# CrispyChillies/Image-Retrieval---Thesis-2026

Measured on AMD Instinct MI355X. Metric: queries/sec (embed+top-10) over 1M x 1024 gallery, higher is better.
Workload: dtype f32 embed (two fp16 MFMA terms); bf16 MFMA candidates + f64 re-rank

## Files before the change

image-retrieval---thesis-2026_amd/csrc/k_conv1x1_h2.hip:

```cpp
#include <atomic>

#include "mirx_device.h"
#include "mirx_kernels.h"

namespace mirx {

namespace {

#ifdef MIRX_C1H2_STAMPS
__device__ unsigned long long g_c1_stamps[8192 * 8];
#define C1_STAMP(ACC)                                                 \
    {                                                                 \
        const unsigned long long now_ = __builtin_amdgcn_s_memtime(); \
        ACC += now_ - st_t;                                           \
        st_t = now_;                                                  \
    }
#else
#define C1_STAMP(ACC)
#endif

constexpr int CM = 128;
constexpr int CP = 128;
constexpr int KC = 16;
constexpr int PLANE_A = CM * KC * 2;
constexpr int PLANE_B = CP * KC * 2;
#ifndef MIRX_C1H2_MIN_WG
#define MIRX_C1H2_MIN_WG 256
#endif
#ifndef MIRX_C1H2_NPT
#define MIRX_C1H2_NPT 2
#endif

__device__ __forceinline__ void pair_exchange(const u32x4 &p, const u32x4 &q, u32x4 &a, u32x4 &b) {
    unsigned a0, a1, a2, a3, b0, b1, b2, b3;
    asm volatile("s_nop 1\n"
                 "s_mov_b64 vcc, %[me]\n"
                 "v_cndmask_b32_dpp %[a0], %[q0], %[p0], vcc quad_perm:[1,0,3,2] row_mask:0xf bank_mask:0xf\n"
                 "v_cndmask_b32_dpp %[a1], %[q1], %[p1], vcc quad_perm:[1,0,3,2] row_mask:0xf bank_mask:0xf\n"
                 "v_cndmask_b32_dpp %[a2], %[q2], %[p2], vcc quad_perm:[1,0,3,2] row_mask:0xf bank_mask:0xf\n"
                 "v_cndmask_b32_dpp %[a3], %[q3], %[p3], vcc quad_perm:[1,0,3,2] row_mask:0xf bank_mask:0xf\n"
                 "s_mov_b64 vcc, %[mo]\n"
                 "v_cndmask_b32_dpp %[b0], %[p0], %[q0], vcc quad_perm:[1,0,3,2] row_mask:0xf bank_mask:0xf\n"
                 "v_cndmask_b32_dpp %[b1], %[p1], %[q1], vcc quad_perm:[1,0,3,2] row_mask:0xf bank_mask:0xf\n"
                 "v_cndmask_b32_dpp %[b2], %[p2], %[q2], vcc quad_perm:[1,0,3,2] row_mask:0xf bank_mask:0xf\n"
                 "v_cndmask_b32_dpp %[b3], %[p3], %[q3], vcc quad_perm:[1,0,3,2] row_mask:0xf bank_mask:0xf\n"
                 : [a0] "=&v"(a0), [a1] "=&v"(a1), [a2] "=&v"(a2), [a3] "=&v"(a3), [b0] "=&v"(b0), [b1] "=&v"(b1),
                   [b2] "=&v"(b2), [b3] "=&v"(b3)
                 : [p0] "v"(p[0]), [p1] "v"(p[1]), [p2] "v"(p[2]), [p3] "v"(p[3]), [q0] "v"(q[0]), [q1] "v"(q[1]),
                   [q2] "v"(q[2]), [q3] "v"(q[3]), [me] "s"(0x5555555555555555ull), [mo] "s"(0xaaaaaaaaaaaaaaaaull)
                 : "vcc");
    a = u32x4{a0, a1, a2, a3};
    b = u32x4{b0, b1, b2, b3};
}

#define C1H2_PARAMS                                                                                                      \
    const float *__restrict__ x, int64_t xbs, int cin, const float *__restrict__ scale, const float *__restrict__ shift, \
        const uint16_t *__restrict__ w2, const float *__restrict__ oscale, const float *__restrict__ bias, int64_t n,     \
        int hw, int cout, float *__restrict__ y, int64_t ybs, const float *__restrict__ in_amax, float in_ks, float in_kb, \
        unsigned *__restrict__ out_amax, float y_ks, float y_kb, float *__restrict__ y_inv_out, int64_t xps, int64_t yps
#define C1H2_ARGS x, xbs, cin, scale, shift, w2, oscale, bias, n, hw, cout, y, ybs, in_amax, in_ks, in_kb, out_amax, y_ks, y_kb, \
                  y_inv_out, xps, yps

template <bool PROLOGUE, bool RELU_OUT, bool YTERMS, int NPT, bool TABLED>
__device__ __forceinline__ void conv1x1_tiled(C1H2_PARAMS) {
    extern __shared__ __attribute__((aligned(16))) char sm[];
    constexpr int KIMG = 8;
    __shared__ float sBias[CM], sOsc[KIMG][CM];
    constexpr bool YFOLD = YTERMS && TABLED;
    __shared__ float sBiasY[YFOLD ? KIMG : 1][CM];
    const int wave = __builtin_amdgcn_readfirstlane(threadIdx.x >> 6), lane = threadIdx.x & 63;
    const int tid = threadIdx.x;
    const int wm = wave >> 1, wn = wave & 1;
    const int64_t total = n * (int64_t)hw;
    constexpr int STAGE_N = 2 * PLANE_A + NPT * 2 * PLANE_B;
    const int64_t p0 = (int64_t)blockIdx.x * (CP * NPT);
    const int co0 = blockIdx.y * CM;
    const int nk = cin / KC;

    auto image_bound = [&](int64_t img) { return fmaf(in_ks, in_amax ? in_amax[img] : 0.f, in_kb); };

    const int b_px = tid & 127;
    const int b_kg = wave >> 1;
    const int64_t in_hw = xps;
    const float *xsrc[NPT];
    float x_scale[NPT];
    unsigned st_img[NPT];
#pragma unroll
    for (int u = 0; u < NPT; ++u) {
        const unsigned pp = (unsigned)(p0 + u * CP + b_px);
        const bool live = pp < (unsigned)total;
        const unsigned pimg = (live ? pp : (unsigned)total - 1u) / (unsigned)hw;
        const int64_t b_off = live ? (int64_t)pimg * xbs + (pp - pimg * (unsigned)hw) : 0;
        st_img[u] = pimg;
        xsrc[u] = x + b_off + (int64_t)(8 * b_kg) * in_hw;
    }
#if defined(MIRX_C1H2_EXP_SKIP) && (MIRX_C1H2_EXP_SKIP & 32)
    const int b_row = b_px;
#else
    const int b_row = YTERMS ? ((b_px & ~31) | ((b_px & 15) << 1) | ((b_px >> 4) & 1)) : b_px;
#endif
    const int b_lds = 2 * PLANE_A + b_row * 32 + ((b_kg ^ ((b_row >> 3) & 1)) << 4);
    const int ep_px = YTERMS ? 16 * (lane & 1) + ((lane & 31) >> 1) : (lane & 31);
    const __amdgpu_buffer_rsrc_t wrsrc = __builtin_amdgcn_make_buffer_rsrc(
        (void *)(w2 + ((int64_t)blockIdx.y * nk) * (2 * CM * KC)), 0, nk * (2 * CM * KC * 2), 0x00020000);
    const int w_voff = (lane >> 1) * 32 + (((lane & 1) ^ ((lane >> 4) & 1)) << 4);
    [[maybe_unused]] auto dma_w1 = [&](int kt, int buf, int i) {
        const int piece = wave + 4 * i;
        __builtin_amdgcn_raw_ptr_buffer_load_lds(wrsrc, LDS_PTR(sm + buf * STAGE_N + piece * 1024), 16, w_voff,
                                                 kt * (2 * CM * KC * 2) + piece * 1024, 0, 0);
    };
    [[maybe_unused]] auto dma_w = [&](int kt, int buf) {
        dma_w1(kt, buf, 0);
        dma_w1(kt, buf, 1);
    };

    constexpr int NR = 8;
    float ra[NPT][NR], rb[NPT][NR], sca[8], sha[8], scb[8], shb[8];
    auto load = [&](int kt, float (&r)[NPT][NR], float (&rsc)[8], float (&rsh)[8]) {
#pragma unroll
        for (int u = 0; u < NPT; ++u)
#pragma unroll
            for (int j = 0; j < 8; ++j) {
                r[u][j] = xsrc[u][((int64_t)kt * KC + j) * in_hw];
            }
        if (PROLOGUE) {
#pragma unroll
            for (int j = 0; j < 8; ++j) {
                rsc[j] = scale[kt * KC + 8 * b_kg + j];
                rsh[j] = shift[kt * KC + 8 * b_kg + j];
            }
        }
    };
#ifdef MIRX_C1H2_STAMPS
    unsigned long long st_t = __builtin_amdgcn_s_memtime(), st_wait = 0, st_bar = 0, st_issue = 0, st_mfma = 0, st_store = 0, st_valu = 0;
    const unsigned long long st_begin = st_t, rt_begin = __builtin_amdgcn_s_memrealtime();
#endif
    auto store = [&](int buf, const float (&r)[NPT][NR], const float (&rsc)[8], const float (&rsh)[8]) {
        char *sb = sm + buf * STAGE_N;
#pragma unroll
        for (int u = 0; u < NPT; ++u) {
            u32x4 ph, pl;
#pragma unroll
            for (int j = 0; j < 4; ++j) {
                f32x2 v;
                v[0] = r[u][2 * j];
                v[1] = r[u][2 * j + 1];
                if (PROLOGUE) {
                    v[0] = fmaxf(fmaf(v[0], rsc[2 * j], rsh[2 * j]), 0.f);
                    v[1] = fmaxf(fmaf(v[1], rsc[2 * j + 1], rsh[2 * j + 1]), 0.f);
                }
                unsigned th, tl;
#if defined(MIRX_C1H2_EXP_SPLIT) && MIRX_C1H2_EXP_SPLIT == 0
                th = __float_as_uint(r[u][2 * j]);
                tl = __float_as_uint(r[u][2 * j + 1]);
#elif defined(MIRX_C1H2_EXP_SPLIT) && MIRX_C1H2_EXP_SPLIT == 1
                th = __float_as_uint(v[0] * x_scale[u]);
                tl = __float_as_uint(v[1] * x_scale[u]);
#else
                split2h_pair(v[0] * x_scale[u], v[1] * x_scale[u], th, tl);
#endif
                ph[j] = th;
                pl[j] = tl;
            }
#ifdef MIRX_C1H2_STAMPS
            if (u == NPT - 1) {
                __builtin_amdgcn_sched_barrier(0);
                asm volatile("s_waitcnt lgkmcnt(0)" ::: "memory");
                C1_STAMP(st_valu)
            }
#endif
            *reinterpret_cast<u32x4 *>(sb + b_lds + u * 2 * PLANE_B) = ph;
            *reinterpret_cast<u32x4 *>(sb + b_lds + u * 2 * PLANE_B + PLANE_B) = pl;
        }
    };

    const int kg = lane >> 5;
    constexpr int NN = 2 * NPT;
    int fa[2], fb[2];
#pragma unroll
    for (int t = 0; t < 2; ++t) {
        const int ra_ = wm * 64 + t * 32 + (lane & 31);
        fa[t] = ra_ * 32 + ((kg ^ ((ra_ >> 3) & 1)) << 4);
        const int rb_ = wn * 64 + t * 32 + (lane & 31);
        fb[t] = 2 * PLANE_A + rb_ * 32 + ((kg ^ ((rb_ >> 3) & 1)) << 4);
    }

    const unsigned img_first = (unsigned)(p0 < total ? p0 : total - 1) / (unsigned)hw;
    const unsigned p_last = (unsigned)(p0 + CP * NPT - 1 < total ? p0 + CP * NPT - 1 : total - 1);
    constexpr bool tabled = TABLED;

    f32x16 acc[2][NN];
#pragma unroll
    for (int mi = 0; mi < 2; ++mi)
#pragma unroll
        for (int ni = 0; ni < NN; ++ni)
#pragma unroll
            for (int r = 0; r < 16; ++r) acc[mi][ni][r] = 0.f;

    auto stage = [&](int kt, int cur, float (&rnext)[NPT][NR], float (&scn)[8], float (&shn)[8], const float (&rstore)[NPT][NR],
                     const float (&scs)[8], const float (&shs)[8]) {
        C1_STAMP(st_store)
        asm volatile("s_waitcnt vmcnt(0)" ::: "memory");
        C1_STAMP(st_wait)
        __syncthreads();
        C1_STAMP(st_bar)
#if defined(MIRX_C1H2_EXP_SKIP) && (MIRX_C1H2_EXP_SKIP & 1)
        if (kt < 0)
#endif
        dma_w(kt + 1 < nk ? kt + 1 : kt, cur ^ 1);
        __builtin_amdgcn_sched_barrier(0);
        load(kt + 2 < nk ? kt + 2 : nk - 1, rnext, scn, shn);
        __builtin_amdgcn_sched_barrier(0);
        C1_STAMP(st_issue)
        const char *sb = sm + cur * STAGE_N;
        f16x8 a[2][2], b[NN][2];
#pragma unroll
        for (int t = 0; t < 2; ++t)
#pragma unroll
            for (int p = 0; p < 2; ++p) a[t][p] = *reinterpret_cast<const f16x8 *>(sb + fa[t] + p * PLANE_A);
#pragma unroll
        for (int ni = 0; ni < NN; ++ni)
#pragma unroll
            for (int p = 0; p < 2; ++p)
                b[ni][p] = *reinterpret_cast<const f16x8 *>(sb + fb[ni & 1] + (ni >> 1) * 2 * PLANE_B + p * PLANE_B);
#pragma unroll
        for (int mi = 0; mi < 2; ++mi) {
#pragma unroll
            for (int ni = 0; ni < NN; ++ni) {
                f32x16 c = acc[mi][ni];
#ifndef MIRX_C1H2_EXP_ONE_MFMA
                c = __builtin_amdgcn_mfma_f32_32x32x16_f16(a[mi][1], b[ni][0], c, 0, 0, 0);
                c = __builtin_amdgcn_mfma_f32_32x32x16_f16(a[mi][0], b[ni][1], c, 0, 0, 0);
#endif
                c = __builtin_amdgcn_mfma_f32_32x32x16_f16(a[mi][0], b[ni][0], c, 0, 0, 0);
                acc[mi][ni] = c;
            }
        }
        C1_STAMP(st_mfma)
        store(cur ^ 1, rstore, scs, shs);
    };
    dma_w(0, 0);
    load(0, ra, sca, sha);
    load(nk > 1 ? 1 : 0, rb, scb, shb);
    if (tid < CM) {
        const float bias_v = bias ? bias[co0 + tid] : 0.f;
        sBias[tid] = bias_v;
        const float osc = oscale[co0 + tid];
        sOsc[0][tid] = osc;
        if (tabled) {
            const unsigned nimg = p_last / (unsigned)hw - img_first + 1;
            for (unsigned k = 0; k < nimg; ++k) {
                float xs_, xi_;
                const float xb_ = image_bound(img_first + k);
                range_scales(xb_, xs_, xi_);
                float ys_ = 1.f, yi_;
                if (YFOLD) range_scales(fmaf(y_ks, xb_, y_kb), ys_, yi_);
                sOsc[k][tid] = osc * xi_ * ys_;
                if (YFOLD) sBiasY[k][tid] = bias_v * ys_;
            }
        }
    }
#pragma unroll
    for (int u = 0; u < NPT; ++u) {
        float inv_;
        range_scales(image_bound(st_img[u]), x_scale[u], inv_);
    }
    float ep_xinv[NN], ep_ys[NN];
    int ep_k[NN];
#pragma unroll
    for (int ni = 0; ni < NN; ++ni) {
        unsigned pp = (unsigned)(p0 + (ni >> 1) * CP + wn * 64 + 32 * (ni & 1) + ep_px);
        if (pp >= (unsigned)total) pp = (unsigned)total - 1u;
        const unsigned pimg = pp / (unsigned)hw;
        const float xb = image_bound(pimg);
        float xs_, yi_;
        range_scales(xb, xs_, ep_xinv[ni]);
        ep_k[ni] = tabled ? (int)(pimg - img_first) : 0;
        if (tabled) ep_xinv[ni] = 1.f;
        ep_ys[ni] = 1.f;
        if (YTERMS) range_scales(fmaf(y_ks, xb, y_kb), ep_ys[ni], yi_);
    }

    store(0, ra, sca, sha);
    int kt = 0;
    for (; kt + 1 < nk; kt += 2) {
        stage(kt, 0, ra, sca, sha, rb, scb, shb);
        stage(kt + 1, 1, rb, scb, shb, ra, sca, sha);
    }
    if (kt < nk) stage(kt, 0, ra, sca, sha, rb, scb, shb);
#ifdef MIRX_C1H2_STAMPS
    if (threadIdx.x == 0) {
        const unsigned long long now_ = __builtin_amdgcn_s_memtime();
        unsigned long long *o = g_c1_stamps + ((blockIdx.x + blockIdx.y * gridDim.x) & 8191) * 8;
        o[0] = now_ - st_begin;
        o[1] = __builtin_amdgcn_s_memrealtime() - rt_begin;
        o[2] = nk;
        o[3] = st_wait;
        o[4] = st_bar;
        o[5] = st_issue;
        o[6] = st_mfma;
        o[7] = (st_store << 32) | (st_valu & 0xffffffffull);
    }
#endif

#if defined(MIRX_C1H2_EXP_SKIP) && (MIRX_C1H2_EXP_SKIP & 2)
    if (in_ks > -1e30f) return;
#endif
    if (YTERMS) {
        uint16_t *yt = reinterpret_cast<uint16_t *>(y);
        auto nb = [](unsigned v) { return (unsigned)__builtin_amdgcn_update_dpp(0, (int)v, 0xB1, 0xf, 0xf, true); };
        const bool even = !(lane & 1);
#pragma unroll
        for (int ni = 0; ni < NN; ++ni) {
            const unsigned pp = (unsigned)(p0 + (ni >> 1) * CP + wn * 64 + 32 * (ni & 1) + ep_px);
            const bool live = pp < (unsigned)total;
            const unsigned ubimg = (live ? pp : 0u) / (unsigned)hw;
            const int64_t bimg = ubimg;
            const unsigned off = pp - ubimg * (unsigned)hw;
            if (live && off == 0 && wm == 0 && lane < 32) {
                float ys_, y_inv;
                range_scales(fmaf(y_ks, image_bound(bimg), y_kb), ys_, y_inv);
                y_inv_out[bimg] = y_inv;
            }
            const unsigned q_own = live ? ubimg * 16u * (unsigned)hw + off : 0xffffffffu;
            const unsigned q_nb = nb(q_own);
            const unsigned qa = even ? q_own : q_nb, qb = even ? q_nb : q_own;
            [[maybe_unused]] const float x_inv = ep_xinv[ni], y_scale = ep_ys[ni];
#pragma unroll
            for (int mi = 0; mi < 2; ++mi) {
                const int g = 4 * wm + 2 * mi + (lane >> 5);
                u32x4 h0, h1, l0, l1;
#pragma unroll
                for (int j = 0; j < 8; ++j) {
                    f32x2 v;
#pragma unroll
                    for (int e = 0; e < 2; ++e) {
                        const int r = 2 * j + e;
                        const int ch = wm * 64 + mi * 32 + (r & 3) + 8 * (r >> 2) + 4 * (lane >> 5);
#if defined(MIRX_C1H2_EXP_SKIP) && (MIRX_C1H2_EXP_SKIP & 8)
                        v[e] = acc[mi][ni][r];
                        (void)ch;
#else
                        float t = fmaf(acc[mi][ni][r], TABLED ? sOsc[ep_k[ni]][ch] : sOsc[0][ch] * x_inv,
                                       YFOLD ? sBiasY[ep_k[ni]][ch] : sBias[ch]);
                        t = __int_as_float(max(__float_as_int(t), 0));
                        v[e] = YFOLD ? t : t * y_scale;
#endif
                    }
                    unsigned hh, ll;
#if defined(MIRX_C1H2_EXP_SKIP) && (MIRX_C1H2_EXP_SKIP & 8)
                    hh = __float_as_uint(v[0]);
                    ll = __float_as_uint(v[1]);
#else
                    split2h_pair(v[0], v[1], hh, ll);
#endif
                    if (j < 4) { h0[j] = hh; l0[j] = ll; }
                    else { h1[j - 4] = hh; l1[j - 4] = ll; }
                }
#if defined(MIRX_C1H2_EXP_SKIP) && (MIRX_C1H2_EXP_SKIP & 4)
                if ((h0[0] ^ h1[1] ^ l0[2] ^ l1[3]) != 0x5a5a1234u) continue;
#endif
                u32x4 ah, al, bh, bl;
                pair_exchange(h0, h1, ah, bh);
                pair_exchange(l0, l1, al, bl);
                const int64_t gofs = (int64_t)(2 * g) * hw;
                const int half = (lane & 1) * 8;
#define C1_ST(P, V) *reinterpret_cast<u32x4 *>(P) = V
                if (qa != 0xffffffffu) {
                    uint16_t *dst = yt + ((int64_t)qa + gofs) * 16 + half;
                    C1_ST(dst, ah);
                    C1_ST(dst + (int64_t)hw * 16, al);
                }
                if (qb != 0xffffffffu) {
                    uint16_t *dst = yt + ((int64_t)qb + gofs) * 16 + half;
                    C1_ST(dst, bh);
                    C1_ST(dst + (int64_t)hw * 16, bl);
                }
#undef C1_ST
            }
        }
        return;
    }
#pragma unroll
    for (int ni = 0; ni < NN; ++ni) {
        unsigned pp = (unsigned)(p0 + (ni >> 1) * CP + wn * 64 + 32 * (ni & 1) + (lane & 31));
        const bool live = pp < (unsigned)total;
        if (!live) pp = (unsigned)total - 1u;
        const unsigned ubimg = pp / (unsigned)hw;
        const int64_t bimg = ubimg, off = pp - ubimg * (unsigned)hw;
        const float x_inv = ep_xinv[ni];
        float vmax = 0.f;
        float *yo = y + bimg * ybs + off;
        if (live) {
#pragma unroll
            for (int mi = 0; mi < 2; ++mi)
#pragma unroll
                for (int r = 0; r < 16; ++r) {
                    const int ch = co0 + wm * 64 + mi * 32 + (r & 3) + 8 * (r >> 2) + 4 * (lane >> 5);
                    float v = fmaf(acc[mi][ni][r], TABLED ? sOsc[ep_k[ni]][ch - co0] : sOsc[0][ch - co0] * x_inv, sBias[ch - co0]);
                    if (RELU_OUT) v = v < 0.f ? 0.f : v;
                    vmax = range_max(vmax, v);
                    yo[(int64_t)ch * yps] = v;
                }
        }
        if (out_amax) range_publish_lanes(out_amax, (int)bimg, vmax, lane);
    }
}

constexpr int RSLOTS = 3;
constexpr int RNP = 2 * CP;
constexpr int RSLOT_W = 2 * PLANE_A;
constexpr int RSLOT = RSLOT_W + KC * RNP * 4;
constexpr int RING_BN = RSLOTS * RSLOT;
constexpr int RING_BN_MAX_CIN = 1024;
constexpr int RING_PIECES = 6;

template <bool PROLOGUE, bool RELU_OUT, bool YTERMS, bool TABLED>
__device__ __forceinline__ void conv1x1_ring(C1H2_PARAMS) {
    extern __shared__ __attribute__((aligned(16))) char sm[];
    constexpr int KIMG = 8;
    constexpr bool YFOLD = YTERMS && TABLED;
    const int wave = __builtin_amdgcn_readfirstlane(threadIdx.x >> 6), lane = threadIdx.x & 63;
    const int tid = threadIdx.x;
    const int64_t total = n * (int64_t)hw;
    const int64_t p0 = (int64_t)blockIdx.x * RNP;
    const int co0 = blockIdx.y * CM;
    const int nk = cin / KC;
    auto image_bound = [&](int64_t img) { return fmaf(in_ks, in_amax ? in_amax[img] : 0.f, in_kb); };
    const unsigned img_first = (unsigned)p0 / (unsigned)hw;
    const unsigned p_last = (unsigned)(p0 + RNP - 1 < total ? p0 + RNP - 1 : total - 1);

    const __amdgpu_buffer_rsrc_t wrsrc = __builtin_amdgcn_make_buffer_rsrc(
        (void *)(w2 + ((int64_t)blockIdx.y * nk) * (2 * CM * KC)), 0, nk * (2 * CM * KC * 2), 0x00020000);
    const int w_voff = (lane >> 1) * 32 + (((lane & 1) ^ ((lane >> 4) & 1)) << 4);
    const __amdgpu_buffer_rsrc_t xrsrc =
        __builtin_amdgcn_make_buffer_rsrc((void *)(x + (int64_t)img_first * xbs), 0, 0x7fffffff, 0x00020000);
    int x_voff = 0;
    {
        const unsigned pp = (unsigned)p0 + 4u * lane;
        if (pp < (unsigned)total) {
            const unsigned pimg = pp / (unsigned)hw;
            x_voff = (int)(((int64_t)(pimg - img_first) * xbs + (pp - pimg * (unsigned)hw)) * 4);
        }
    }
    const int xps4 = (int)xps * 4;
    auto dma = [&](int kt, int slot) {
        char *sb = sm + slot * RSLOT;
#pragma unroll
        for (int i = 0; i < 2; ++i) {
            const int piece = wave + 4 * i;
            __builtin_amdgcn_raw_ptr_buffer_load_lds(wrsrc, LDS_PTR(sb + piece * 1024), 16, w_voff,
                                                     kt * (2 * CM * KC * 2) + piece * 1024, 0, 0);
        }
#pragma unroll
        for (int i = 0; i < 4; ++i) {
            const int c = 4 * wave + i;
            __builtin_amdgcn_raw_ptr_buffer_load_lds(xrsrc, LDS_PTR(sb + RSLOT_W + c * (RNP * 4)), 16, x_voff,
                                                     (kt * KC + c) * xps4, 0, 0);
        }
    };

    float *bn = reinterpret_cast<float *>(sm + RING_BN);
    constexpr int BNR = PROLOGUE ? 2 * RING_BN_MAX_CIN / 256 : 1;
    float bnv[BNR];
    if (PROLOGUE) {
#pragma unroll
        for (int i = 0; i < BNR; ++i) {
            const int e = tid + 256 * i;
            bnv[i] = e < cin ? scale[e] : (e < 2 * cin ? shift[e - cin] : 0.f);
        }
    }
    float t_bias = 0.f, t_osc = 0.f;
    if (tid < CM) {
        t_bias = bias ? bias[co0 + tid] : 0.f;
        t_osc = oscale[co0 + tid];
    }
    const unsigned nimg = p_last / (unsigned)hw - img_first + 1;
    __builtin_amdgcn_sched_barrier(0);
    dma(0, 0);
    if (nk > 1) dma(1, 1);
    __builtin_amdgcn_sched_barrier(0);
    if (PROLOGUE) {
#pragma unroll
        for (int i = 0; i < BNR; ++i) {
            const int e = tid + 256 * i;
            if (e < 2 * cin) bn[e] = bnv[i];
        }
    }
    float ib[KIMG];
#pragma unroll
    for (int k = 0; k < KIMG; ++k) ib[k] = TABLED && (unsigned)k < nimg ? image_bound(img_first + k) : 0.f;

    const int ep_px = YTERMS ? 16 * (lane & 1) + ((lane & 31) >> 1) : (lane & 31);
    float x_scale[2], ep_xinv[2], ep_ys[2];
    int ep_k[2];
#pragma unroll
    for (int ni = 0; ni < 2; ++ni) {
        unsigned pp = (unsigned)(p0 + 64 * wave + 32 * ni + ep_px);
        if (pp >= (unsigned)total) pp = (unsigned)total - 1u;
        const unsigned pimg = pp / (unsigned)hw;
        const float xb = image_bound(pimg);
        float yi_;
        range_scales(xb, x_scale[ni], ep_xinv[ni]);
        ep_k[ni] = TABLED ? (int)(pimg - img_first) : 0;
        if (TABLED) ep_xinv[ni] = 1.f;
        ep_ys[ni] = 1.f;
        if (YTERMS) range_scales(fmaf(y_ks, xb, y_kb), ep_ys[ni], yi_);
    }

    const int kg = lane >> 5;
    int fa[4];
#pragma unroll
    for (int mi = 0; mi < 4; ++mi) {
        const int ra_ = mi * 32 + (lane & 31);
        fa[mi] = ra_ * 32 + ((kg ^ ((ra_ >> 3) & 1)) << 4);
    }
    const int fb = RSLOT_W + 8 * kg * (RNP * 4) + (64 * wave + ep_px) * 4;

    f32x16 acc[4][2];
#pragma unroll
    for (int mi = 0; mi < 4; ++mi)
#pragma unroll
        for (int ni = 0; ni < 2; ++ni)
#pragma unroll
            for (int r = 0; r < 16; ++r) acc[mi][ni][r] = 0.f;

    int slot = 0;
    for (int kt = 0; kt < nk; ++kt) {
        if (kt + 1 < nk) asm volatile("s_waitcnt vmcnt(%0)" ::"n"(RING_PIECES) : "memory");
        else asm volatile("s_waitcnt vmcnt(0)" ::: "memory");
        asm volatile("s_waitcnt lgkmcnt(0)\n\ts_barrier" ::: "memory");
        if (kt + 2 < nk) dma(kt + 2, slot == 0 ? 2 : slot - 1);
        __builtin_amdgcn_sched_barrier(0);
        const char *sb = sm + slot * RSLOT;
        f16x8 a[4][2], b[2][2];
#pragma unroll
        for (int mi = 0; mi < 4; ++mi)
#pragma unroll
            for (int p = 0; p < 2; ++p) a[mi][p] = *reinterpret_cast<const f16x8 *>(sb + fa[mi] + p * PLANE_A);
        float sc[8], sh[8];
        if (PROLOGUE) {
#pragma unroll
            for (int j = 0; j < 8; ++j) {
                sc[j] = bn[kt * KC + 8 * kg + j];
                sh[j] = bn[cin + kt * KC + 8 * kg + j];
            }
        }
#pragma unroll
        for (int ni = 0; ni < 2; ++ni) {
            u32x4 ph, pl;
#pragma unroll
            for (int j = 0; j < 4; ++j) {
                f32x2 v;
                v[0] = *reinterpret_cast<const float *>(sb + fb + (2 * j) * (RNP * 4) + ni * 128);
                v[1] = *reinterpret_cast<const float *>(sb + fb + (2 * j + 1) * (RNP * 4) + ni * 128);
                if (PROLOGUE) {
                    v[0] = fmaxf(fmaf(v[0], sc[2 * j], sh[2 * j]), 0.f);
                    v[1] = fmaxf(fmaf(v[1], sc[2 * j + 1], sh[2 * j + 1]), 0.f);
                }
                unsigned th, tl;
                split2h_pair(v[0] * x_scale[ni], v[1] * x_scale[ni], th, tl);
                ph[j] = th;
                pl[j] = tl;
            }
            b[ni][0] = __builtin_bit_cast(f16x8, ph);
            b[ni][1] = __builtin_bit_cast(f16x8, pl);
        }
#pragma unroll
        for (int mi = 0; mi < 4; ++mi) {
#pragma unroll
            for (int ni = 0; ni < 2; ++ni) {
                f32x16 c = acc[mi][ni];
                c = __builtin_amdgcn_mfma_f32_32x32x16_f16(a[mi][1], b[ni][0], c, 0, 0, 0);
                c = __builtin_amdgcn_mfma_f32_32x32x16_f16(a[mi][0], b[ni][1], c, 0, 0, 0);
                c = __builtin_amdgcn_mfma_f32_32x32x16_f16(a[mi][0], b[ni][0], c, 0, 0, 0);
                acc[mi][ni] = c;
            }
        }
        slot = slot == RSLOTS - 1 ? 0 : slot + 1;
    }

    float *sBias = reinterpret_cast<float *>(sm + (nk % RSLOTS) * RSLOT);
    float(*sOsc)[CM] = reinterpret_cast<float(*)[CM]>(sBias + CM);
    float(*sBiasY)[CM] = reinterpret_cast<float(*)[CM]>(sBias + CM + KIMG * CM);
    if (tid < CM) {
        sBias[tid] = t_bias;
        sOsc[0][tid] = t_osc;
        if (TABLED) {
#pragma unroll
            for (int k = 0; k < KIMG; ++k) {
                if ((unsigned)k < nimg) {
                    float xs_, xi_;
                    range_scales(ib[k], xs_, xi_);
                    float ys_ = 1.f, yi_;
                    if (YFOLD) range_scales(fmaf(y_ks, ib[k], y_kb), ys_, yi_);
                    sOsc[k][tid] = t_osc * xi_ * ys_;
                    if (YFOLD) sBiasY[k][tid] = t_bias * ys_;
                }
            }
        }
    }
    asm volatile("s_waitcnt lgkmcnt(0)\n\ts_barrier" ::: "memory");

    if (YTERMS) {
        uint16_t *yt = reinterpret_cast<uint16_t *>(y);
        auto nb = [](unsigned v) { return (unsigned)__builtin_amdgcn_update_dpp(0, (int)v, 0xB1, 0xf, 0xf, true); };
        const bool even = !(lane & 1);
#pragma unroll
        for (int ni = 0; ni < 2; ++ni) {
            const unsigned pp = (unsigned)(p0 + 64 * wave + 32 * ni + ep_px);
            const bool live = pp < (unsigned)total;
            const unsigned ubimg = (live ? pp : 0u) / (unsigned)hw;
            const int64_t bimg = ubimg;
            const unsigned off = pp - ubimg * (unsigned)hw;
            if (live && off == 0 && lane < 32) {
                float ys_, y_inv;
                range_scales(fmaf(y_ks, image_bound(bimg), y_kb), ys_, y_inv);
                y_inv_out[bimg] = y_inv;
            }
            const unsigned q_own = live ? ubimg * 16u * (unsigned)hw + off : 0xffffffffu;
            const unsigned q_nb = nb(q_own);
            const unsigned qa = even ? q_own : q_nb, qb = even ? q_nb : q_own;
            [[maybe_unused]] const float x_inv = ep_xinv[ni], y_scale = ep_ys[ni];
#pragma unroll
            for (int mi = 0; mi < 4; ++mi) {
                const int g = 2 * mi + (lane >> 5);
                u32x4 h0, h1, l0, l1;
#pragma unroll
                for (int j = 0; j < 8; ++j) {
                    f32x2 v;
#pragma unroll
                    for (int e = 0; e < 2; ++e) {
                        const int r = 2 * j + e;
                        const int ch = mi * 32 + (r & 3) + 8 * (r >> 2) + 4 * (lane >> 5);
                        float t = fmaf(acc[mi][ni][r], TABLED ? sOsc[ep_k[ni]][ch] : sOsc[0][ch] * x_inv,
                                       YFOLD ? sBiasY[ep_k[ni]][ch] : sBias[ch]);
                        t = __int_as_float(max(__float_as_int(t), 0));
                        v[e] = YFOLD ? t : t * y_scale;
                    }
                    unsigned hh, ll;
                    split2h_pair(v[0], v[1], hh, ll);
                    if (j < 4) { h0[j] = hh; l0[j] = ll; }
                    else { h1[j - 4] = hh; l1[j - 4] = ll; }
                }
                u32x4 ah, al, bh, bl;
                pair_exchange(h0, h1, ah, bh);
                pair_exchange(l0, l1, al, bl);
                const int64_t gofs = (int64_t)(2 * g) * hw;
                const int half = (lane & 1) * 8;
                if (qa != 0xffffffffu) {
                    uint16_t *dst = yt + ((int64_t)qa + gofs) * 16 + half;
                    *reinterpret_cast<u32x4 *>(dst) = ah;
                    *reinterpret_cast<u32x4 *>(dst + (int64_t)hw * 16) = al;
                }
                if (qb != 0xffffffffu) {
                    uint16_t *dst = yt + ((int64_t)qb + gofs) * 16 + half;
                    *reinterpret_cast<u32x4 *>(dst) = bh;
                    *reinterpret_cast<u32x4 *>(dst + (int64_t)hw * 16) = bl;
                }
            }
        }
        return;
    }
#pragma unroll
    for (int ni = 0; ni < 2; ++ni) {
        unsigned pp = (unsigned)(p0 + 64 * wave + 32 * ni + (lane & 31));
        const bool live = pp < (unsigned)total;
        if (!live) pp = (unsigned)total - 1u;
        const unsigned ubimg = pp / (unsigned)hw;
        const int64_t bimg = ubimg, off = pp - ubimg * (unsigned)hw;
        const float x_inv = ep_xinv[ni];
        float vmax = 0.f;
        float *yo = y + bimg * ybs + off;
        if (live) {
#pragma unroll
            for (int mi = 0; mi < 4; ++mi)
#pragma unroll
                for (int r = 0; r < 16; ++r) {
                    const int ch = mi * 32 + (r & 3) + 8 * (r >> 2) + 4 * (lane >> 5);
                    float v = fmaf(acc[mi][ni][r], TABLED ? sOsc[ep_k[ni]][ch] : sOsc[0][ch] * x_inv, sBias[ch]);
                    if (RELU_OUT) v = v < 0.f ? 0.f : v;
                    vmax = range_max(vmax, v);
                    yo[(int64_t)(co0 + ch) * yps] = v;
                }
        }
        if (out_amax) range_publish_lanes(out_amax, (int)bimg, vmax, lane);
    }
}

template <bool PROLOGUE, bool RELU_OUT, bool YTERMS, int NPT, bool TABLED, bool RING>
__global__ __launch_bounds__(256, NPT == 2 ? 2 : 3) void k_conv1x1_h2(C1H2_PARAMS) {
    if constexpr (RING) conv1x1_ring<PROLOGUE, RELU_OUT, YTERMS, TABLED>(C1H2_ARGS);
    else conv1x1_tiled<PROLOGUE, RELU_OUT, YTERMS, NPT, TABLED>(C1H2_ARGS);
}

}

#ifdef MIRX_C1H2_STAMPS
extern "C" int mirx_debug_c1_stamps(unsigned long long *out) {
    return (int)hipMemcpyFromSymbol(out, HIP_SYMBOL(g_c1_stamps), sizeof(g_c1_stamps));
}
#endif

static std::atomic<int> g_small_max_wg{128};
void set_conv1x1_small_max_wg(int v) { g_small_max_wg.store(v < 0 ? 0 : v); }
static int conv1x1_small_max_wg() { return g_small_max_wg.load(std::memory_order_relaxed); }
static std::atomic<int> g_ring{1};
void set_conv1x1_ring(int v) { g_ring.store(v ? 1 : 0); }
static bool conv1x1_ring_enabled() { return g_ring.load(std::memory_order_relaxed) != 0; }

hipError_t launch_conv1x1_h2(const float *x, int64_t xbs, int cin, const float *scale, const float *shift,
                             const uint16_t *w2, const float *oscale, const float *bias, int64_t n, int hw, int cout,
                             int relu_out, float *y, int64_t ybs, const float *in_amax, float in_ks, float in_kb,
                             float *out_amax, float y_ks, float y_kb, float *y_inv_out, int64_t xps, int64_t yps,
                             hipStream_t st) {
    if (n <= 0) return hipSuccess;
    if (cin % KC || cout % CM || !oscale) return hipErrorInvalidValue;
    const bool yterms = y_inv_out != nullptr;
    if (yterms && (cout != CM || !relu_out || !scale)) return hipErrorInvalidValue;
    if (!xps) xps = hw;
    if (!yps) yps = hw;
    if (xps < hw || yps < hw) return hipErrorInvalidValue;
    const int64_t px = n * (int64_t)hw;
    if (px >= ((int64_t)1 << 31) - 2 * CP) return hipErrorInvalidValue;
    if (yterms && px >= ((int64_t)1 << 27)) return hipErrorInvalidValue;
    const bool small_bn_ok = !scale || (cin <= 1024 && ((reinterpret_cast<uintptr_t>(scale) | reinterpret_cast<uintptr_t>(shift)) & 15) == 0);
    if (px * (cout / CM) < (int64_t)CP * conv1x1_small_max_wg() && small_bn_ok)
        return launch_conv1x1_h2_small(x, xbs, cin, scale, shift, w2, oscale, bias, n, hw, cout, relu_out, y, ybs, in_amax,
                                       in_ks, in_kb, out_amax, y_ks, y_kb, y_inv_out, xps, yps, st);
    const int npt = px >= (int64_t)2 * CP * MIRX_C1H2_MIN_WG ? MIRX_C1H2_NPT : 1;
    const bool ring = npt == 2 && conv1x1_ring_enabled() && hw % 4 == 0 && xps % 4 == 0 && xbs % 4 == 0 &&
                      (reinterpret_cast<uintptr_t>(x) & 15) == 0 && (!scale || cin <= RING_BN_MAX_CIN) &&
                      ((int64_t)((RNP - 1) / hw + 2) * xbs + (int64_t)cin * xps) * 4 < ((int64_t)1 << 31);
    const dim3 grid((unsigned)((px + CP * npt - 1) / (CP * npt)), (unsigned)(cout / CM));
    const size_t lds = ring ? (size_t)RING_BN + (scale ? (size_t)cin * 8 : 0) : 2 * (size_t)(2 * PLANE_A + npt * 2 * PLANE_B);
    unsigned *oa = reinterpret_cast<unsigned *>(out_amax);
    const bool tabled = (CP * npt - 1) / hw + 2 <= 8;
#define MIRX_H2K(P, R, T, N, RG)                                                                           \
    {                                                                                                      \
        if (tabled) MIRX_H2KT(P, R, T, N, true, RG) else MIRX_H2KT(P, R, T, N, false, RG)                  \
    }
#define MIRX_H2KT(P, R, T, N, TB, RG)                                                                      \
    {                                                                                                      \
        static std::atomic<unsigned long long> attr_devs{0};       \
        hipError_t e = set_dynamic_lds(k_conv1x1_h2<P, R, T, N, TB, RG>, RG ? RING_BN + 8 * RING_BN_MAX_CIN : 2 * (2 * PLANE_A + N * 2 * PLANE_B), &attr_devs);    \
        if (e != hipSuccess) return e;                                                                 \
        hipLaunchKernelGGL((k_conv1x1_h2<P, R, T, N, TB, RG>), grid, dim3(256), lds, st, x, xbs, cin, scale, shift, w2, oscale, \
                           bias, n, hw, cout, y, ybs, in_amax, in_ks, in_kb, oa, y_ks, y_kb, y_inv_out, xps, yps); \
    }
#define MIRX_H2C(P, R, T)                                                                                  \
    {                                                                                                      \
        if (ring) MIRX_H2K(P, R, T, 2, true) else if (npt == 2) MIRX_H2K(P, R, T, 2, false) else MIRX_H2K(P, R, T, 1, false) \
    }
    if (yterms) {
        MIRX_H2C(true, true, true)
    } else if (scale) {
        if (relu_out) MIRX_H2C(true, true, false) else MIRX_H2C(true, false, false)
    } else {
        if (relu_out) MIRX_H2C(false, true, false) else MIRX_H2C(false, false, false)
    }
#undef MIRX_H2K
#undef MIRX_H2KT
#undef MIRX_H2C
    return hipGetLastError();
}

}
```

Measured before the change: 43760.

## Software-pipeline fp16 split conversion of next K-tile under current MFMAs

Splits the LDS DMA into separate weight and activation loads. Activations are now fetched one K-step ahead of the weights, into a shifted ring slot. The loop is restructured so the next tile's activation loads from LDS, optional BN/ReLU prologue and hi/lo fp16 split are interleaved between the MFMA groups of the current tile, with ping-pong B-fragment registers. This is meant to hide the VALU conversion latency behind matrix-core work, at the cost of more live registers and more delicate vmcnt accounting. Optional timing stamps are added behind a compile flag.

```diff
diff --git a/image-retrieval---thesis-2026_amd/csrc/k_conv1x1_h2.hip b/image-retrieval---thesis-2026_amd/csrc/k_conv1x1_h2.hip
--- a/image-retrieval---thesis-2026_amd/csrc/k_conv1x1_h2.hip
+++ b/image-retrieval---thesis-2026_amd/csrc/k_conv1x1_h2.hip
@@ -1,4 +1,5 @@
 #include <atomic>
+#include <type_traits>
 
 #include "mirx_device.h"
 #include "mirx_kernels.h"
@@ -444,20 +445,25 @@
         }
     }
     const int xps4 = (int)xps * 4;
-    auto dma = [&](int kt, int slot) {
-        char *sb = sm + slot * RSLOT;
+    auto dma_w = [&](int kt, int slot) {
 #pragma unroll
         for (int i = 0; i < 2; ++i) {
             const int piece = wave + 4 * i;
-            __builtin_amdgcn_raw_ptr_buffer_load_lds(wrsrc, LDS_PTR(sb + piece * 1024), 16, w_voff,
+            __builtin_amdgcn_raw_ptr_buffer_load_lds(wrsrc, LDS_PTR(sm + slot * RSLOT + piece * 1024), 16, w_voff,
                                                      kt * (2 * CM * KC * 2) + piece * 1024, 0, 0);
         }
+    };
+    auto dma_x = [&](int kt, int slot) {
 #pragma unroll
         for (int i = 0; i < 4; ++i) {
             const int c = 4 * wave + i;
-            __builtin_amdgcn_raw_ptr_buffer_load_lds(xrsrc, LDS_PTR(sb + RSLOT_W + c * (RNP * 4)), 16, x_voff,
+            __builtin_amdgcn_raw_ptr_buffer_load_lds(xrsrc, LDS_PTR(sm + slot * RSLOT + RSLOT_W + c * (RNP * 4)), 16, x_voff,
                                                      (kt * KC + c) * xps4, 0, 0);
         }
+    };
+    auto dma = [&](int v, int slot) {
+        dma_w(v, slot);
+        if (v + 1 < nk) dma_x(v + 1, slot);
     };
 
     float *bn = reinterpret_cast<float *>(sm + RING_BN);
@@ -477,6 +483,7 @@
     }
     const unsigned nimg = p_last / (unsigned)hw - img_first + 1;
     __builtin_amdgcn_sched_barrier(0);
+    dma_x(0, 2);
     dma(0, 0);
     if (nk > 1) dma(1, 1);
     __builtin_amdgcn_sched_barrier(0);
@@ -525,60 +532,137 @@
 #pragma unroll
             for (int r = 0; r < 16; ++r) acc[mi][ni][r] = 0.f;
 
-    int slot = 0;
-    for (int kt = 0; kt < nk; ++kt) {
-        if (kt + 1 < nk) asm volatile("s_waitcnt vmcnt(%0)" ::"n"(RING_PIECES) : "memory");
-        else asm volatile("s_waitcnt vmcnt(0)" ::: "memory");
+#ifdef MIRX_C1H2_STAMPS
+    unsigned long long st_t = __builtin_amdgcn_s_memtime(), st_wait = 0, st_bar = 0, st_issue = 0, st_pre = 0, st_mfma = 0;
+    const unsigned long long st_begin = st_t, rt_begin = __builtin_amdgcn_s_memrealtime();
+#endif
+    struct raw_t {
+        float v[2][8], sc[8], sh[8];
+    };
+    auto fetch = [&](const char *sb, int kt, raw_t &r) {
+        if (PROLOGUE) {
+#pragma unroll
+            for (int j = 0; j < 8; ++j) {
+                r.sc[j] = bn[kt * KC + 8 * kg + j];
+                r.sh[j] = bn[cin + kt * KC + 8 * kg + j];
+            }
+        }
+#pragma unroll
+        for (int ni = 0; ni < 2; ++ni)
+#pragma unroll
+            for (int j = 0; j < 8; ++j) r.v[ni][j] = *reinterpret_cast<const float *>(sb + fb + j * (RNP * 4) + ni * 128);
+    };
+    auto split_col = [&](const raw_t &r, int ni, f16x8 (&b)[2][2]) {
+        u32x4 ph, pl;
+#pragma unroll
+        for (int j = 0; j < 4; ++j) {
+            f32x2 v;
+            v[0] = r.v[ni][2 * j];
+            v[1] = r.v[ni][2 * j + 1];
+            if (PROLOGUE) {
+                v[0] = fmaxf(fmaf(v[0], r.sc[2 * j], r.sh[2 * j]), 0.f);
+                v[1] = fmaxf(fmaf(v[1], r.sc[2 * j + 1], r.sh[2 * j + 1]), 0.f);
+            }
+            unsigned th, tl;
+            split2h_pair(v[0] * x_scale[ni], v[1] * x_scale[ni], th, tl);
+            ph[j] = th;
+            pl[j] = tl;
+        }
+        b[ni][0] = __builtin_bit_cast(f16x8, ph);
+        b[ni][1] = __builtin_bit_cast(f16x8, pl);
+    };
+    auto convert = [&](const char *sb, int kt, f16x8 (&b)[2][2]) {
+        raw_t r;
+        fetch(sb, kt, r);
+        split_col(r, 0, b);
+        split_col(r, 1, b);
+    };
+    auto stage = [&](auto next_tag, int kt, int slot, const f16x8 (&bc)[2][2], f16x8 (&bn_)[2][2]) {
+        constexpr bool NEXT = decltype(next_tag)::value;
+        if (!NEXT) asm volatile("s_waitcnt vmcnt(0)" ::: "memory");
+        else if (kt + 2 < nk) asm volatile("s_waitcnt vmcnt(%0)" ::"n"(RING_PIECES) : "memory");
+        else asm volatile("s_waitcnt vmcnt(2)" ::: "memory");
+        C1_STAMP(st_wait)
         asm volatile("s_waitcnt lgkmcnt(0)\n\ts_barrier" ::: "memory");
+        C1_STAMP(st_bar)
         if (kt + 2 < nk) dma(kt + 2, slot == 0 ? 2 : slot - 1);
         __builtin_amdgcn_sched_barrier(0);
+        C1_STAMP(st_issue)
         const char *sb = sm + slot * RSLOT;
-        f16x8 a[4][2], b[2][2];
+        f16x8 a[4][2];
 #pragma unroll
         for (int mi = 0; mi < 4; ++mi)
 #pragma unroll
             for (int p = 0; p < 2; ++p) a[mi][p] = *reinterpret_cast<const f16x8 *>(sb + fa[mi] + p * PLANE_A);
-        float sc[8], sh[8];
-        if (PROLOGUE) {
-#pragma unroll
-            for (int j = 0; j < 8; ++j) {
-                sc[j] = bn[kt * KC + 8 * kg + j];
-                sh[j] = bn[cin + kt * KC + 8 * kg + j];
-            }
-        }
-#pragma unroll
-        for (int ni = 0; ni < 2; ++ni) {
-            u32x4 ph, pl;
-#pragma unroll
-            for (int j = 0; j < 4; ++j) {
-                f32x2 v;
-                v[0] = *reinterpret_cast<const float *>(sb + fb + (2 * j) * (RNP * 4) + ni * 128);
-                v[1] = *reinterpret_cast<const float *>(sb + fb + (2 * j + 1) * (RNP * 4) + ni * 128);
-                if (PROLOGUE) {
-                    v[0] = fmaxf(fmaf(v[0], sc[2 * j], sh[2 * j]), 0.f);
-                    v[1] = fmaxf(fmaf(v[1], sc[2 * j + 1], sh[2 * j + 1]), 0.f);
-                }
-                unsigned th, tl;
-                split2h_pair(v[0] * x_scale[ni], v[1] * x_scale[ni], th, tl);
-                ph[j] = th;
-                pl[j] = tl;
-            }
-            b[ni][0] = __builtin_bit_cast(f16x8, ph);
-            b[ni][1] = __builtin_bit_cast(f16x8, pl);
-        }
+#ifdef MIRX_C1H2_STAMPS
+        __builtin_amdgcn_sched_barrier(0);
+        asm volatile("s_waitcnt lgkmcnt(0)" ::: "memory");
+        C1_STAMP(st_pre)
+#endif
+        raw_t r;
+        if (NEXT) fetch(sb, kt + 1, r);
 #pragma unroll
         for (int mi = 0; mi < 4; ++mi) {
+            if (NEXT && (mi == 1 || mi == 2)) split_col(r, mi - 1, bn_);
 #pragma unroll
             for (int ni = 0; ni < 2; ++ni) {
                 f32x16 c = acc[mi][ni];
-                c = __builtin_amdgcn_mfma_f32_32x32x16_f16(a[mi][1], b[ni][0], c, 0, 0, 0);
-                c = __builtin_amdgcn_mfma_f32_32x32x16_f16(a[mi][0], b[ni][1], c, 0, 0, 0);
-                c = __builtin_amdgcn_mfma_f32_32x32x16_f16(a[mi][0], b[ni][0], c, 0, 0, 0);
+                c = __builtin_amdgcn_mfma_f32_32x32x16_f16(a[mi][1], bc[ni][0], c, 0, 0, 0);
+                c = __builtin_amdgcn_mfma_f32_32x32x16_f16(a[mi][0], bc[ni][1], c, 0, 0, 0);
+                c = __builtin_amdgcn_mfma_f32_32x32x16_f16(a[mi][0], bc[ni][0], c, 0, 0, 0);
                 acc[mi][ni] = c;
             }
-        }
+            if (NEXT && mi < 3) __builtin_amdgcn_sched_barrier(0);
+        }
+#ifdef MIRX_C1H2_STAMPS
+        __builtin_amdgcn_sched_barrier(0);
+        C1_STAMP(st_mfma)
+#endif
+    };
+    using next_t = std::integral_constant<bool, true>;
+    using last_t = std::integral_constant<bool, false>;
+
+    if (nk > 2) asm volatile("s_waitcnt vmcnt(%0)" ::"n"(2 * RING_PIECES) : "memory");
+    else if (nk == 2) asm volatile("s_waitcnt vmcnt(%0)" ::"n"(RING_PIECES + 2) : "memory");
+    else asm volatile("s_waitcnt vmcnt(2)" ::: "memory");
+    asm volatile("s_waitcnt lgkmcnt(0)\n\ts_barrier" ::: "memory");
+    f16x8 b[2][2], bnext[2][2];
+    convert(sm + 2 * RSLOT, 0, b);
+    C1_STAMP(st_pre)
+    int kt = 0, slot = 0;
+    auto advance = [&]() {
+        ++kt;
         slot = slot == RSLOTS - 1 ? 0 : slot + 1;
-    }
+    };
+    while (kt + 2 < nk) {
+        stage(next_t{}, kt, slot, b, bnext);
+        advance();
+        stage(next_t{}, kt, slot, bnext, b);
+        advance();
+    }
+    if (kt + 1 < nk) {
+        stage(next_t{}, kt, slot, b, bnext);
+        advance();
+#pragma unroll
+        for (int ni = 0; ni < 2; ++ni)
+#pragma unroll
+            for (int p = 0; p < 2; ++p) b[ni][p] = bnext[ni][p];
+    }
+    stage(last_t{}, kt, slot, b, bnext);
+#ifdef MIRX_C1H2_STAMPS
+    if (threadIdx.x == 0) {
+        const unsigned long long now_ = __builtin_amdgcn_s_memtime();
+        unsigned long long *o = g_c1_stamps + ((blockIdx.x + blockIdx.y * gridDim.x) & 8191) * 8;
+        o[0] = now_ - st_begin;
+        o[1] = __builtin_amdgcn_s_memrealtime() - rt_begin;
+        o[2] = (unsigned long long)nk | (1ull << 32);
+        o[3] = st_wait;
+        o[4] = st_bar;
+        o[5] = st_issue;
+        o[6] = st_mfma;
+        o[7] = st_pre;
+    }
+#endif
 
     float *sBias = reinterpret_cast<float *>(sm + (nk % RSLOTS) * RSLOT);
     float(*sOsc)[CM] = reinterpret_cast<float(*)[CM]>(sBias + CM);
```

Measured after the change: 43540. No clear change (-0.5%).
